# eezkni/UEGAN

Measured on AMD Instinct MI355X. Metric: train imgs/sec @512px bs=16 on 1/2/4/8 MI355X; infer ms/img, higher is better.
Workload: dtype bf16; 1 GPU; FiveK-shaped 512x512 batch=16/GPU, full G/D/VGG train step (trainer.py:77-119), conv_dim=32, seeded stand-in VGG19; global_batch=16, parallelism=dp1, pool_size=50, collective=none (1 rank), passes=batched (fused.py)

## Files before the change

uegan_amd/csrc/conv_core.h:

```cpp
#pragma once
#include "common.h"
#include "conv_internal.h"

#include <stdio.h>
#include <stdlib.h>
#include <utility>
#include <vector>

namespace uegan {

struct ProfRecord {
  hipEvent_t start, stop;
  int kernel_id;
  double flops, bytes;
};
extern bool g_prof_on;
extern std::vector<ProfRecord> g_prof_records;
extern std::vector<std::pair<hipEvent_t, hipEvent_t>> g_prof_pool;
extern size_t g_prof_used;

static inline int prof_key(int kind, bool bf16, int bn, int ks, int mode, int th, bool glds) {
  return (kind << 28) | ((bf16 ? 1 : 0) << 24) | (bn << 12) | (ks << 8) | (mode << 4) | ((th == 32 ? 2 : (th == 16 ? 1 : (th == 4 ? 3 : 0))) << 1) | (glds ? 1 : 0);
}
static void prof_kernel_name(int key, char* buf, size_t n) {
// ... 106 lines not shown
    if (o < out_n - 1 - g.pad || o > out_n - 2) return -1;
    pp = 2 * (out_n - 1) - o;
  }
  const int t2 = pp + g.pad - t;
  if (t2 < 0) return -1;
  int s = t2;
  if (g.stride == 2) {
    if (t2 & 1) return -1;
    s = t2 >> 1;
  }
  return s < in_n ? s : -1;
}

__device__ __forceinline__ bool has_image(const ConvGeom& g, int o, int img, int out_n) {
  if (img == 0) return true;
  if (g.mode == 0 || g.pad_mode != UEGAN_PAD_REFLECT) return false;
  if (img == 1) return o >= 1 && o <= g.pad;
  return o >= out_n - 1 - g.pad && o <= out_n - 2;
}

__device__ __forceinline__ int swz128(int r) { return ((r >> 1) & 3) << 1; }
__device__ __forceinline__ int swz64(int r) { return ((r >> 2) & 1) << 1; }

static __device__ __attribute__((aligned(16))) const unsigned int g_zero16[4] = {0u, 0u, 0u, 0u};

__device__ __forceinline__ void glds16(const void* gsrc, void* lds_wave_base) {
  __builtin_amdgcn_global_load_lds((const __attribute__((address_space(1))) void*)gsrc,
                                   (__attribute__((address_space(3))) void*)lds_wave_base, 16, 0, 0);
}

__device__ __forceinline__ void wgtr_glds16(const unsigned char* base, uint32_t off, unsigned char* lds_wave_base) {
#ifdef UEGAN_EMU
  glds16(base + off, lds_wave_base);
#else
  const uint32_t dst = (uint32_t)(uintptr_t)(__attribute__((address_space(3))) unsigned char*)lds_wave_base;
  uint32_t keep;
  asm volatile("s_mov_b32 %0, m0\n\ts_mov_b32 m0, %3\n\ts_nop 0\n\tglobal_load_lds_dwordx4 %1, %2\n\ts_mov_b32 m0, %0"
               : "=&s"(keep) : "v"(off), "s"(base), "s"(dst) : "memory");
#endif
}
__device__ __forceinline__ void wgtr_glds16(const void* src, unsigned char* lds_wave_base) {
#ifdef UEGAN_EMU
  glds16(src, lds_wave_base);
#else
  const uint32_t dst = (uint32_t)(uintptr_t)(__attribute__((address_space(3))) unsigned char*)lds_wave_base;
  uint32_t keep;
  asm volatile("s_mov_b32 %0, m0\n\ts_mov_b32 m0, %2\n\ts_nop 0\n\tglobal_load_lds_dwordx4 %1, off\n\ts_mov_b32 m0, %0"
               : "=&s"(keep) : "v"(src), "s"(dst) : "memory");
#endif
}
__device__ __forceinline__ void wgtr_wait_loads() {
#ifndef UEGAN_EMU
  asm volatile("s_waitcnt vmcnt(0)" ::: "memory");
#endif
}

struct ConvArgs {
  ConvGeom g;
  const void* in1;
  const void* in2;
  const void* w;
  const float* bias;
  const float* scale;
  int scale_group;
  void* out;
  void* out2;
  int n_out1;
  int N, Kp, act, nbias;
  int nty, ntx;
  int frame;
  int fy0, fy1, fx0, fx1;
  const void* mask;
  int mask_act;
  void* pool_out = nullptr;
  int pool_done = 0;
  void* pool_idx = nullptr;
  int n_idx = 0;
  int n_full = 1 << 30;
  int xcd_map = 0;
  int rect_y0 = 0, rect_y1 = 0, rect_x0 = 0, rect_x1 = 0;
  int border_only = 0;
  float* stats_part = nullptr;
  int stats_tpi = 0;
  const void* in1_lo = nullptr;
  const void* in2_lo = nullptr;
  const void* w_lo = nullptr;
  void* out_lo = nullptr;
  const void* mul = nullptr;
  const void* mul_lo = nullptr;
  void* out_mul = nullptr;
  void* out_mul_lo = nullptr;
  int src_wrap = 0;
  const float* res_x = nullptr;
  const float* res_x2 = nullptr;
  float* res_out = nullptr;
  float* res_out2 = nullptr;
  int res_split = 1 << 30;
  float* kws = nullptr;
  size_t kws_bytes = 0;
  int kparts = 0, kchunks = 0;
};

static inline int splitk_parts(const ConvArgs& a, int blocks, int nchunk, int* kchunks) {
  *kchunks = nchunk;
  if (!a.kws || a.g.mode != 0 || a.frame || a.out2 || a.mask || a.pool_out || a.stats_part || a.out_lo || a.mul || a.res_out || blocks <= 0) return 1;
  int parts = 1;
// ... 16 lines not shown
```

uegan_amd/csrc/conv_stream.h:

```cpp
#pragma once

struct ConvStreamArgs {
  ConvArgs c;
  int flip;
  int org;
  int zero_fill;
  int cls;
  int kstart[5];
  int ymin;
  int sx;
  int TH, PW, PH, PWmagic, KWmagic;
  int rb, rblog, Clog;
  int ksteps, taps;
  int wrow, wrows;
  int wbytes, tbytes, xbytes;
  int mtab_off;
  int xmir;
  int ty0, ty1, tx0, tx1;
  int tiles_total, tiles_per_block;
  int abl;
  int lo_xoff, c_lo, rb_lo, rblog_lo, wlo_off, tlo_off;
};

__device__ __forceinline__ int cs_swz(int rb, int pcol) {
  return rb == 128 ? swz128(pcol) : (rb == 64 ? swz64(pcol) : 0);
}

constexpr int CS_LDS_KB[4] = {53, 80, 152, 160};

template <int TN, int PF, int LC, bool CLS, bool XMIR = false, int NW = 4, bool STATS = false, int PR = 0, int EPX = 0>
__global__ void __launch_bounds__(64 * NW, (LC >= 2 ? 1 : (LC == 1 ? 2 : 3)) * NW / 4) conv_stream_kernel(ConvStreamArgs a) {
  constexpr int NT = 64 * NW;
  constexpr int MAXIX = (LC >= 2 ? 16 : 10) * 4 / NW;
  constexpr bool WLO = PR >= 1;
  static_assert(PR == 0 || (!CLS && !XMIR), "hi + lo pairs: plain forward only");
  __shared__ __attribute__((aligned(16))) unsigned char lds[CS_LDS_KB[LC] * 1024];
  const ConvArgs& ca = a.c;
  const ConvGeom& g = ca.g;
  const unsigned char* in1 = static_cast<const unsigned char*>(ca.in1);
  const unsigned char* in2 = static_cast<const unsigned char*>(ca.in2);
  const int tid = threadIdx.x, lane = tid & 63;
  const int wave = __builtin_amdgcn_readfirstlane(tid >> 6);
  const int fj = lane & 15, fg = lane >> 4;
  unsigned char* wl = lds;
  unsigned char* tab = lds + a.wbytes;
  unsigned char* xb0 = tab + a.tbytes;

  if (XMIR) {
    int* mflag = reinterpret_cast<int*>(tab + a.mtab_off) + 2 * a.ksteps * 64;
    for (int i = tid; i < 2 * a.ksteps; i += NT) mflag[i] = 0;
    __syncthreads();
  }
  {
    const int cpr = a.ksteps * 4;
    const int total = a.wrows * cpr;
    const bf16_t* w = static_cast<const bf16_t*>(ca.w);
    for (int idx = tid; idx < total; idx += NT) {
      const int n = idx / cpr, q = idx - n * cpr;
      u32x4 v = u32x4{0u, 0u, 0u, 0u};
      if (n < ca.N && q * 8 < ca.Kp) v = *reinterpret_cast<const u32x4*>(w + (size_t)n * ca.Kp + q * 8);
      *reinterpret_cast<u32x4*>(wl + n * a.wrow + (q >> 2) * 64 + (((q & 3) ^ swz64(n)) << 4)) = v;
      if constexpr (WLO) {
        u32x4 vl = u32x4{0u, 0u, 0u, 0u};
        if (n < ca.N && q * 8 < ca.Kp) vl = *reinterpret_cast<const u32x4*>(static_cast<const bf16_t*>(ca.w_lo) + (size_t)n * ca.Kp + q * 8);
        *reinterpret_cast<u32x4*>(wl + a.wlo_off + n * a.wrow + (q >> 2) * 64 + (((q & 3) ^ swz64(n)) << 4)) = vl;
      }
    }
    int* tab2 = reinterpret_cast<int*>(tab + a.ksteps * 256);
    if (!CLS) {
      for (int idx = tid; idx < a.ksteps * 64; idx += NT) {
        const int s = idx >> 6, l = idx & 63;
        const int k = 32 * s + 8 * (l >> 4);
        int tap = k >> a.Clog;
        const int chunk = (k & ((1 << a.Clog) - 1)) >> 3;
        if (tap >= a.taps) tap = 0;
        int ty = (tap * a.KWmagic) >> 16, tx = tap - ty * g.KW;
        if (a.flip) { ty = g.KH - 1 - ty; tx = g.KW - 1 - tx; }
        const int pcol = a.sx * (l & 15) + tx;
        *reinterpret_cast<int*>(tab + idx * 4) = (ty * a.PW + pcol) * a.rb + ((chunk ^ cs_swz(a.rb, pcol)) << 4);
        if (l == 0) tab2[s] = s * 64;
        if (XMIR) {
// ... 50 lines not shown
  const int nxc = (a.PH * a.PW) << cprlog;
  const int cprlog_lo = PR >= 2 ? a.rblog_lo - 4 : 0;
  const int nlo0 = PR >= 2 ? a.lo_xoff >> 4 : 0, nxcl = PR >= 2 ? (a.PH * a.PW) << cprlog_lo : 0;
  const int nix = PR >= 2 ? (nlo0 + nxcl + NT - 1) / NT : (nxc + NT - 1) / NT;
  const unsigned char* in_lo = PR == 2 ? static_cast<const unsigned char*>(ca.in1_lo) : (PR == 3 ? static_cast<const unsigned char*>(ca.in2_lo) : nullptr);
  const bool two_src = g.C2 != 0;
  auto decode = [&](int L, int& prow, int& pcol, int& c, int& sel) -> bool {
    if (PR >= 2 && L >= nlo0) {
      const int L2 = L - nlo0;
      if (L2 >= nxcl) return false;
      const int r = L2 >> cprlog_lo, pos = L2 & ((1 << cprlog_lo) - 1);
      prow = (r * a.PWmagic) >> 16; pcol = r - prow * a.PW;
      c = (pos ^ cs_swz(a.rb_lo, pcol)) << 3;
      sel = 2;
      return true;
    }
    if (PR >= 2 && L >= nxc) return false;
    const int r = L >> cprlog, pos = L & ((1 << cprlog) - 1);
    prow = (r * a.PWmagic) >> 16; pcol = r - prow * a.PW;
    c = (pos ^ cs_swz(a.rb, pcol)) << 3;
    sel = c < g.C1 ? 0 : 1;
    if (sel) c -= g.C1;
    return true;
  };
  uint32_t xoff[MAXIX];
#pragma unroll
  for (int it = 0; it < MAXIX; ++it) {
    const int L = it * NT + tid;
    xoff[it] = PR >= 2 ? 0xffffffffu : 0u;
    int prow, pcol, c, sel;
    if (L < (PR >= 2 ? nlo0 + nxcl : nxc) && decode(L, prow, pcol, c, sel)) {
      if (sel == 0) xoff[it] = (uint32_t)(((prow * g.IW + pcol) * g.C1 + c) * 2);
      else if (sel == 1) xoff[it] = (uint32_t)(((prow * g.IW + pcol) * g.C2 + c) * 2) | 0x80000000u;
      else xoff[it] = (uint32_t)(((prow * g.IW + pcol) * a.c_lo + c) * 2) | 0x40000000u;
    }
  }
  int abase[TN];
#pragma unroll
  for (int nf = 0; nf < TN; ++nf) {
    int n = nf * 16 + fj;
    if (n >= a.wrows) n -= a.wrows;
    abase[nf] = n * a.wrow + ((fg ^ swz64(n)) << 4);
  }
  float bv[TN][4];
#pragma unroll
  for (int nf = 0; nf < TN; ++nf)
#pragma unroll
    for (int r = 0; r < 4; ++r) {
      const int n = nf * 16 + fg * 4 + r;
      bv[nf][r] = (ca.bias && n < ca.nbias) ? ca.bias[n] : 0.f;
    }
  __syncthreads();

  const int nrx = a.tx1 - a.tx0, nry = a.ty1 - a.ty0;
  int t_begin = blockIdx.x * a.tiles_per_block, t_end = t_begin + a.tiles_per_block;
  if (t_end > a.tiles_total) t_end = a.tiles_total;

  auto tile_origin = [&](int t, int& b, int& oy0, int& ox0) {
    const int txi = t % nrx;
    const int tq = t / nrx;
    const int tyi = tq % nry;
    b = tq / nry;
    oy0 = (a.ty0 + tyi) * a.TH;
    ox0 = (a.tx0 + txi) * 16;
  };

  auto stage = [&](int t, int bufi) {
    unsigned char* xb = xb0 + bufi * a.xbytes;
    int b, oy0, ox0;
    tile_origin(t, b, oy0, ox0);
    const int iy0 = CLS ? oy0 + a.ymin : a.sx * oy0 + a.org, ix0 = CLS ? ox0 + a.ymin : a.sx * ox0 + a.org;
    const bool inside = iy0 >= 0 && iy0 + a.PH <= g.IH && ix0 >= 0 && ix0 + a.PW <= g.IW;
    if (inside) {
      const long long pix0 = ((long long)b * g.IH + iy0) * g.IW + ix0;
      const unsigned char* o1 = in1 + pix0 * g.C1 * 2;
      const unsigned char* o2 = in2 + pix0 * g.C2 * 2;
      const unsigned char* o3 = PR >= 2 ? in_lo + pix0 * a.c_lo * 2 : nullptr;
#pragma unroll
      for (int it = 0; it < MAXIX; ++it)
        if (it < nix) {
          const uint32_t o = xoff[it];
          unsigned char* dst = xb + (it * NT + wave * 64) * 16;
          if (PR >= 2 && o == 0xffffffffu) continue;
          if (PR >= 2 && (o & 0x40000000u)) wgtr_glds16(o3, o & 0x3fffffffu, dst);
          else if (two_src && (o >> 31)) wgtr_glds16(o2, o & 0x7fffffffu, dst);
          else wgtr_glds16(o1, o, dst);
        }
    } else if (!a.zero_fill) {
      const long long img = (long long)b * g.IH * g.IW;
      const unsigned char* o1 = in1 + img * g.C1 * 2;
      const unsigned char* o2 = in2 + img * g.C2 * 2;
      const unsigned char* o3 = PR >= 2 ? in_lo + img * a.c_lo * 2 : nullptr;
#pragma unroll 1
      for (int it = 0; it < nix; ++it) {
        const int L = it * NT + tid;
        int prow, pcol, c, sel;
        unsigned char* dst = xb + (it * NT + wave * 64) * 16;
        if (!decode(L, prow, pcol, c, sel)) continue;
        int iy = iy0 + prow, ix = ix0 + pcol;
        iy = iy < 0 ? -iy : iy;
        iy = iy >= g.IH ? 2 * (g.IH - 1) - iy : iy;
        iy = iy < 0 ? 0 : (iy >= g.IH ? g.IH - 1 : iy);
        ix = ix < 0 ? -ix : ix;
        ix = ix >= g.IW ? 2 * (g.IW - 1) - ix : ix;
        ix = ix < 0 ? 0 : (ix >= g.IW ? g.IW - 1 : ix);
        const uint32_t pix = (uint32_t)(iy * g.IW + ix);
        if (sel == 0) wgtr_glds16(o1, (pix * (uint32_t)g.C1 + (uint32_t)c) * 2u, dst);
        else if (sel == 1) wgtr_glds16(o2, (pix * (uint32_t)g.C2 + (uint32_t)c) * 2u, dst);
        else wgtr_glds16(o3, (pix * (uint32_t)a.c_lo + (uint32_t)c) * 2u, dst);
      }
    } else {
#pragma unroll 1
      for (int it = 0; it < nix; ++it) {
        const int L = it * NT + tid;
        const void* src = g_zero16;
        if (L < nxc) {
          const int r = L >> cprlog, pos = L & ((1 << cprlog) - 1);
          const int prow = (r * a.PWmagic) >> 16, pcol = r - prow * a.PW;
          const int c = (pos ^ cs_swz(a.rb, pcol)) << 3;
          const int iy = iy0 + prow, ix = ix0 + pcol;
          if (iy >= 0 && iy < g.IH && ix >= 0 && ix < g.IW) {
            const long long pix = ((long long)b * g.IH + iy) * g.IW + ix;
            src = c < g.C1 ? in1 + (pix * g.C1 + c) * 2 : in2 + (pix * g.C2 + (c - g.C1)) * 2;
          }
        }
        wgtr_glds16(src, xb + (it * NT + wave * 64) * 16);
      }
    }
  };

  bf16_t* out = static_cast<bf16_t*>(ca.out);
  float st1[STATS ? TN : 1][4], st2[STATS ? TN : 1][4];
  int st_b = -1;
  const int st_b0 = STATS ? t_begin / (ca.stats_tpi > 0 ? ca.stats_tpi : 1) : 0;
  if (STATS) {
#pragma unroll
    for (int nf = 0; nf < TN; ++nf)
#pragma unroll
      for (int r = 0; r < 4; ++r) { st1[nf][r] = 0.f; st2[nf][r] = 0.f; }
  }
  auto stats_flush = [&](int bimg) {
    if constexpr (STATS) {
      float* dst = ca.stats_part + ((size_t)((blockIdx.x * 2 + (bimg - st_b0)) * NW + wave) * (TN * 16)) * 2;
#pragma unroll
      for (int nf = 0; nf < TN; ++nf)
#pragma unroll
        for (int r = 0; r < 4; ++r) {
          float a1 = st1[nf][r], a2 = st2[nf][r];
#pragma unroll
          for (int o = 1; o < 16; o <<= 1) { a1 += __shfl_xor(a1, o, 64); a2 += __shfl_xor(a2, o, 64); }
          if (fj == 0) { dst[(nf * 16 + fg * 4 + r) * 2] = a1; dst[(nf * 16 + fg * 4 + r) * 2 + 1] = a2; }
          st1[nf][r] = 0.f; st2[nf][r] = 0.f;
        }
    }
  };
  const int row0 = wave * PF;
  int sc_grp = -1;
  float scale = 1.f;
  const int rowpitch = a.sx * a.PW * a.rb;
  for (int t = t_begin - 1; t < t_end; ++t) {
    const bool have = t >= t_begin;
    const int bufi = (t - t_begin) & 1;
    if (have) {
      wgtr_wait_loads();
      raw_barrier();
    }
    if (t + 1 < t_end && !((UEGAN_ABL_BITS(a.abl) & 1) && have)) stage(t + 1, bufi ^ 1);
    if (!have) continue;
    const unsigned char* xw = xb0 + bufi * a.xbytes + row0 * rowpitch;
    const int* tab2 = reinterpret_cast<const int*>(tab + a.ksteps * 256);
    constexpr int ncls = CLS ? 4 : 1;
   for (int cl = 0; cl < ncls; ++cl) {
    const int ks0 = CLS ? a.kstart[cl] : 0, ks1 = CLS ? a.kstart[cl + 1] : a.ksteps;
    f32x4 acc[TN][PF];
#pragma unroll
    for (int nf = 0; nf < TN; ++nf)
#pragma unroll
      for (int i = 0; i < PF; ++i) acc[nf][i] = f32x4{0.f, 0.f, 0.f, 0.f};
    u32x2 mulh[EPX == 2 ? TN : 1][EPX == 2 ? PF : 1], mull[EPX == 2 ? TN : 1][EPX == 2 ? PF : 1];
    if constexpr (EPX == 2) {
      int bq, oyq, oxq;
      tile_origin(t, bq, oyq, oxq);
#pragma unroll
      for (int i = 0; i < PF; ++i) {
        const int oy = oyq + row0 + i, oxp = oxq + fj;
        const bool pvq = oy < g.OH && oxp < g.OW;
        const size_t pq = ((size_t)bq * g.OH + oy) * g.OW + oxp;
#pragma unroll
        for (int nf = 0; nf < TN; ++nf) {
          mulh[nf][i] = u32x2{0u, 0u}; mull[nf][i] = u32x2{0u, 0u};
          if (pvq && nf * 16 + fg * 4 < ca.N) {
            const size_t eo = pq * ca.N + nf * 16 + fg * 4;
            mulh[nf][i] = *reinterpret_cast<const u32x2*>(static_cast<const bf16_t*>(ca.mul) + eo);
            if (ca.mul_lo) mull[nf][i] = *reinterpret_cast<const u32x2*>(static_cast<const bf16_t*>(ca.mul_lo) + eo);
          }
        }
      }
    }
    u32x4 a0[TN], b0[PF], a1[TN], b1[PF];
   if constexpr (PR != 0) {
    const int rowpitch_lo = a.sx * a.PW * a.rb_lo;
    const unsigned char* xwl = xb0 + bufi * a.xbytes + a.lo_xoff + row0 * rowpitch_lo;
    u32x4 al0[TN], al1[TN], bl0[PF], bl1[PF];
    auto load_p = [&](int s, auto odd_c, u32x4 (&af)[TN], u32x4 (&afl)[TN], u32x4 (&bf)[PF], u32x4 (&bfl)[PF]) {
      constexpr bool ODD = decltype(odd_c)::value;
      const int boff = *reinterpret_cast<const int*>(tab + (s * 64 + lane) * 4);
#pragma unroll
      for (int nf = 0; nf < TN; ++nf) {
        af[nf] = *reinterpret_cast<const u32x4*>(wl + abase[nf] + s * 64);
        afl[nf] = *reinterpret_cast<const u32x4*>(wl + a.wlo_off + abase[nf] + s * 64);
      }
#pragma unroll
      for (int i = 0; i < PF; ++i) bf[i] = *reinterpret_cast<const u32x4*>(xw + boff + i * rowpitch);
      if constexpr (PR == 2) {
#pragma unroll
        for (int i = 0; i < PF; ++i) bfl[i] = *reinterpret_cast<const u32x4*>(xwl + boff + i * rowpitch_lo);
      }
      if constexpr (PR == 3 && ODD) {
        const int bl = *reinterpret_cast<const int*>(tab + a.tlo_off + ((s >> 1) * 64 + lane) * 4);
#pragma unroll
        for (int i = 0; i < PF; ++i) bfl[i] = *reinterpret_cast<const u32x4*>(xwl + bl + i * rowpitch_lo);
      }
    };
    auto mma_p = [&](auto odd_c, const u32x4 (&af)[TN], const u32x4 (&afl)[TN], const u32x4 (&bf)[PF], const u32x4 (&bfl)[PF]) {
      constexpr bool ODD = decltype(odd_c)::value;
#pragma unroll
      for (int nf = 0; nf < TN; ++nf)
#pragma unroll
        for (int i = 0; i < PF; ++i) {
          if constexpr (PR == 2 || (PR == 3 && ODD)) acc[nf][i] = mfma_bf16(af[nf], bfl[i], acc[nf][i]);
          acc[nf][i] = mfma_bf16(afl[nf], bf[i], acc[nf][i]);
          acc[nf][i] = mfma_bf16(af[nf], bf[i], acc[nf][i]);
        }
    };
    const std::false_type even_c{};
    const std::true_type odd_c{};
    load_p(0, even_c, a0, al0, b0, bl0);
    for (int s = 0; s < ks1; s += 2) {
      if (s + 1 < ks1) load_p(s + 1, odd_c, a1, al1, b1, bl1);
      mma_p(even_c, a0, al0, b0, bl0);
      if (s + 1 >= ks1) break;
      if (s + 2 < ks1) load_p(s + 2, even_c, a0, al0, b0, bl0);
      mma_p(odd_c, a1, al1, b1, bl1);
    }
   } else {
    int boff_nx = *reinterpret_cast<const int*>(tab + (ks0 * 64 + lane) * 4);
    auto load_frags = [&](int s, u32x4 (&af)[TN], u32x4 (&bf)[PF]) {
      const int boff = boff_nx;
      if (s + 1 < ks1) boff_nx = *reinterpret_cast<const int*>(tab + ((s + 1) * 64 + lane) * 4);
      const int aoff = CLS ? tab2[s] : s * 64;
#pragma unroll
      for (int nf = 0; nf < TN; ++nf) af[nf] = *reinterpret_cast<const u32x4*>(wl + abase[nf] + aoff);
#pragma unroll
      for (int i = 0; i < PF; ++i) bf[i] = *reinterpret_cast<const u32x4*>(xw + boff + i * rowpitch);
    };
// ... 232 lines not shown
  int cspan = 0;
  for (int c = 0; c < 5; ++c) a.kstart[c] = 0;
  if (cls) {
    const int ymin = (g.pad & 1) ? (1 - g.pad) / 2 : -(g.pad / 2);
    int ymax = 0;
    for (int py = 0; py < 2; ++py) {
      const int t0 = (py + g.pad) & 1, v = (py + g.pad - t0) / 2;
      if (v > ymax) ymax = v;
    }
    a.ymin = ymin;
    cspan = ymax - ymin;
    a.PW = 16 + cspan;
    const int spt = g.C / 32;
    for (int c = 0; c < 4; ++c) {
      const int py = c >> 1, px = c & 1;
      const int nty = (g.KH - ((py + g.pad) & 1) + 1) / 2, ntx = (g.KW - ((px + g.pad) & 1) + 1) / 2;
      a.kstart[c + 1] = a.kstart[c] + nty * ntx * spt;
    }
    if (a.kstart[4] != a.ksteps) return false;
  }
  a.PWmagic = 65536 / a.PW + 1;
  p.pf = 0;
  p.lc = 1;
  for (int pass = 1; pass < (pr == 3 ? 4 : 3) && !p.pf; ++pass) {
    const int kb = CS_LDS_KB[pass], maxix = pass >= 2 ? 16 : 10;
    for (int pf : {4, 2}) {
      if (pf > max_pf) continue;
      const int th = 4 * pf, ph = cls ? th + cspan : sx * (th - 1) + g.KH;
      const int xbh = pr >= 2 ? ph * a.PW * a.rb : (ph * a.PW * a.rb + 4095) / 4096 * 4096;
      const int xb = xbh + (pr >= 2 ? ph * a.PW * a.rb_lo : 0);
      if (a.wbytes + a.tbytes + 2 * xb > kb * 1024 || (xb + 4095) / 4096 > maxix) continue;
      bool ok = true;
      for (int r = 0; r < ph * a.PW && ok; ++r) ok = ((r * a.PWmagic) >> 16) == r / a.PW;
      if (!ok) continue;
      p.pf = pf; a.TH = th; a.PH = ph; a.xbytes = xb; p.lc = pass;
      if (pr >= 2) a.lo_xoff = xbh;
      break;
    }
  }
  if (!p.pf) return false;
  p.nw = 4;
  if (p.pf == 4 && (!cls || p.lc == 2) && p.lc == 2 && p.tn <= 2 && !a.xmir && !pr) {
    const int xb8 = (a.PH * a.PW * a.rb + 8191) / 8192 * 8192;
    if (a.wbytes + a.tbytes + 2 * xb8 <= CS_LDS_KB[p.lc] * 1024 && xb8 / 8192 <= (p.lc == 2 ? 8 : 5)) { p.nw = 8; p.pf = 2; a.xbytes = xb8; }
  }
  if (pr >= 2 && p.lc >= 2 && p.tn <= 2 && (a.xbytes + 8191) / 8192 <= 8) { p.nw = 8; p.pf /= 2; }
  if (p.lc == 2 && ((p.tn == 4 && sx == 1) || (cls && p.nw != 8))) return false;
  p.fixup = g.mode == 1 && g.pad_mode == UEGAN_PAD_REFLECT && g.pad > 0;
  if (p.fixup && (g.OH <= 2 * g.pad + 2 || g.OW <= 2 * g.pad + 2)) return false;
  a.ty0 = 0; a.tx0 = 0;
  a.ty1 = ((cls ? g.IH : g.OH) + a.TH - 1) / a.TH;
  a.tx1 = ((cls ? g.IW : g.OW) + 15) / 16;
  a.tiles_total = g.B * (a.ty1 - a.ty0) * (a.tx1 - a.tx0);
  const int maxb = p.lc == 2 ? 256 : 512;
  int blocks = a.tiles_total < maxb ? a.tiles_total : maxb;
  a.tiles_per_block = (a.tiles_total + blocks - 1) / blocks;
  p.blocks = (a.tiles_total + a.tiles_per_block - 1) / a.tiles_per_block;
  if ((pr || epx) && !conv_stream_ex_available(p)) return false;
  return true;
}

template <int TN, int PF>
static void conv_stream_launch2(const ConvStreamPlan& p, hipStream_t s) {
  const int blocks = p.blocks;
  if (p.a.cls) {
    if constexpr (PF == 2 && TN <= 2) {
      if (p.nw == 8) {
        hipLaunchKernelGGL((conv_stream_kernel<TN, PF, 2, true, false, 8>), dim3(blocks), dim3(512), 0, s, p.a);
        return;
      }
    }
    if (p.lc == 2) hipLaunchKernelGGL((conv_stream_kernel<TN, PF, 2, true>), dim3(blocks), dim3(256), 0, s, p.a);
    else hipLaunchKernelGGL((conv_stream_kernel<TN, PF, 1, true>), dim3(blocks), dim3(256), 0, s, p.a);
    return;
  }
  if constexpr (PF == 2 && TN <= 2) {
    if (p.nw == 8) {
      if (p.a.xmir) hipLaunchKernelGGL((conv_stream_kernel<TN, PF, 1, false, true, 8>), dim3(blocks), dim3(512), 0, s, p.a);
      else if (p.lc == 2) hipLaunchKernelGGL((conv_stream_kernel<TN, PF, 2, false, false, 8>), dim3(blocks), dim3(512), 0, s, p.a);
      else hipLaunchKernelGGL((conv_stream_kernel<TN, PF, 1, false, false, 8>), dim3(blocks), dim3(512), 0, s, p.a);
      return;
    }
  }
  if (p.stats) {
    if constexpr (TN >= 2) {
      hipLaunchKernelGGL((conv_stream_kernel<TN, PF, 1, false, false, 4, true>), dim3(blocks), dim3(256), 0, s, p.a);
      return;
    }
  }
  if (p.a.xmir) {
    if (p.lc == 2) hipLaunchKernelGGL((conv_stream_kernel<TN, PF, 2, false, true>), dim3(blocks), dim3(256), 0, s, p.a);
    else hipLaunchKernelGGL((conv_stream_kernel<TN, PF, 1, false, true>), dim3(blocks), dim3(256), 0, s, p.a);
    return;
  }
  if (p.lc == 2) hipLaunchKernelGGL((conv_stream_kernel<TN, PF, 2, false>), dim3(blocks), dim3(256), 0, s, p.a);
  else hipLaunchKernelGGL((conv_stream_kernel<TN, PF, 1, false>), dim3(blocks), dim3(256), 0, s, p.a);
}
static bool conv_stream_stats_ok(const ConvStreamPlan& p) {
  const ConvGeom& g = p.a.c.g;
  const int tpi = (p.a.ty1 - p.a.ty0) * (p.a.tx1 - p.a.tx0);
  return g.mode == 0 && !p.a.cls && !p.a.xmir && p.nw == 4 && p.lc == 1 && !p.a.c.out2 && !p.a.c.mask && p.a.tiles_per_block <= tpi && p.tn >= 2;
}
static void conv_stream_launch(const ConvStreamPlan& p, hipStream_t s) {
  if (p.pr || p.epx) {
    (void)conv_stream_launch_ex(p, s);
    return;
// ... 10 lines not shown
```

uegan_amd/csrc/wgrad_tr.h:

```cpp
#pragma once

struct WgradTrArgs {
  ConvGeom g;
  const void* in1;
  const void* in2;
  const void* dz;
  float* ws;
  int N, zC, ktot, pstride, want_bias;
  int TW, TWlog, TH, PW, PWmagic, PWused, nks, dyk;
  int xrb, xrblog, zrb, zrblog;
  int xcb;
  int cfpc, fslots, fpb, nfr;
  int WK, WS;
  int tiles_x, tiles_y, tiles_total, tiles_per_split;
  int xbytes, zbytes;
  int rs;
  int nbuf;
  int xcd_map;
  int abl;
  int head, hE, hEB, hEBlog;
};

__device__ __forceinline__ int wgtr_swz(int rb, int r) {
  return rb == 128 ? (r & 6) : (rb == 64 ? ((r >> 1) & 2) : 0);
}

template <int KB>
__device__ __forceinline__ unsigned char* wgtr_lds() {
  __shared__ __attribute__((aligned(16))) unsigned char buf[KB * 1024];
  return buf;
}

__device__ __forceinline__ u32x2 lds_read_tr16(const unsigned char* p) {
  typedef short v4s_t __attribute__((ext_vector_type(4)));
  const v4s_t r = __builtin_amdgcn_ds_read_tr16_b64_v4i16((__attribute__((address_space(3))) v4s_t*)p);
  return __builtin_bit_cast(u32x2, r);
}

constexpr int WGTR_SMALL_KB = 80, WGTR_BIG_KB = 152;


template <int TN, int TM, bool BIG, bool HEAD>
__global__ void __launch_bounds__(256, BIG ? 1 : 2) wgrad_tr_kernel(WgradTrArgs a) {
  constexpr int MAXIX = BIG ? 19 : 10, MAXIZ = 8;
  unsigned char* lds = wgtr_lds<BIG ? WGTR_BIG_KB : WGTR_SMALL_KB>();
  const ConvGeom& g = a.g;
  const unsigned char* in1 = static_cast<const unsigned char*>(a.in1);
  const unsigned char* in2 = static_cast<const unsigned char*>(a.in2);
  const unsigned char* dz = static_cast<const unsigned char*>(a.dz);
  const int tid = threadIdx.x, lane = tid & 63;
  const int wave = __builtin_amdgcn_readfirstlane(tid >> 6);
  const int wk = wave % a.WK, wsid = wave / a.WK;
  int bx = blockIdx.x, by = blockIdx.y, bz = blockIdx.z;
  if (a.xcd_map) {
    const int P = gridDim.x * gridDim.y, G = a.xcd_map, m = 8 / G;
    const int L = blockIdx.x + gridDim.x * (blockIdx.y + gridDim.y * blockIdx.z);
    const int run = L / (G * P), r = L - run * G * P;
    const int xcd = r & 7, k = r >> 3;
    bz = run * G + xcd % G;
    const int q = k * m + xcd / G;
    by = q / gridDim.x;
    bx = q - by * gridDim.x;
  }
  const int cc = bx / a.nfr, fr = bx - cc * a.nfr;
  const int nb = by, split = bz;
  const int taps = g.KH * g.KW;
  const int f0 = fr * a.fpb;
  int tapA, tapB;
  if (a.cfpc) { tapA = f0 / a.cfpc; tapB = (f0 + a.fpb - 1) / a.cfpc; }
  else { tapA = 2 * f0; tapB = 2 * (f0 + a.fpb) - 1; }
  if (HEAD) { tapA *= g.KW; tapB = tapB * g.KW + g.KW - 1; }
  if (tapB > taps - 1) tapB = taps - 1;
  if (tapA > taps - 1) tapA = taps - 1;
  const int ty_lo = tapA / g.KW, ty_hi = tapB / g.KW;
  const int rstep = g.stride / a.rs;
  const int PH = (a.TH - 1) * rstep + (ty_hi - ty_lo) + 1;
  const int xcpr_log = a.xrblog - 4, zcpr_log = a.zrblog - 4;
  const int nxc = (PH * a.PW) << xcpr_log, nzc = (a.TH * a.TW) << zcpr_log;
  const int c_chunk0 = cc * 64, n_chunk0 = nb * 64;
  const int nix = (nxc + 255) >> 8, niz = (nzc + 255) >> 8;

  uint32_t xoff[MAXIX];
  const bool two_src = g.C2 != 0 && c_chunk0 < g.C1 && c_chunk0 + a.xcb > g.C1;
  const bool chunk_in2 = g.C2 != 0 && c_chunk0 >= g.C1;
#pragma unroll
  for (int it = 0; it < MAXIX; ++it) {
    const int L = it * 256 + tid;
    xoff[it] = 0;
    if (L < nxc) {
      const int r = L >> xcpr_log, pos = L & ((1 << xcpr_log) - 1);
      const int prow = (r * a.PWmagic) >> 16, pcol = r - prow * a.PW;
      const int c = c_chunk0 + ((pos ^ wgtr_swz(a.xrb, pcol)) << 3);
      if (pcol < a.PWused && c < g.C) {
        if (c < g.C1) xoff[it] = (uint32_t)(((prow * a.rs * g.IW + pcol) * g.C1 + c) * 2);
        else xoff[it] = (uint32_t)(((prow * a.rs * g.IW + pcol) * g.C2 + (c - g.C1)) * 2) | (two_src ? 0x80000000u : 0u);
      }
    }
  }
  uint32_t zoff[MAXIZ];
#pragma unroll
  for (int it = 0; it < MAXIZ; ++it) {
    const int L = it * 256 + tid;
    zoff[it] = 0;
    if (L < nzc) {
      const int r = L >> zcpr_log, pos = L & ((1 << zcpr_log) - 1);
      const int oy = r >> a.TWlog, ox = r & (a.TW - 1);
      const int c = n_chunk0 + ((pos ^ wgtr_swz(a.zrb, r)) << 3);
      if (c < a.zC) zoff[it] = (uint32_t)(((oy * g.OW + ox) * a.zC + c) * 2);
    }
  }

  const int g4 = lane >> 4, sj = (lane & 15) >> 2, seg = lane & 3;
  const int dx = sj + 4 * (g4 & 1) + (a.TW == 32 ? 16 * (g4 >> 1) : 0);
  const int dy = a.TW == 32 ? 0 : (g4 >> 1);
  int zaddr[TN], xaddr[TM], xaddr1[TM];
  if (HEAD) {
    const int zch = a.hEB >> 1;
#pragma unroll
    for (int nf = 0; nf < TN; ++nf) {
      int ch = nf * 16 + 4 * seg;
      if (ch >= zch) ch = 4 * (seg & 1);
      zaddr[nf] = dx * a.hEB + ((((ch >> 3) ^ wgtr_swz(a.hEB, dx))) << 4) + ((ch >> 2) & 1) * 8;
    }
#pragma unroll
    for (int m = 0; m < TM; ++m) {
      const int f = f0 + wk * TM + m;
      int ty = f / a.cfpc;
      const int ch = (f - ty * a.cfpc) * 16 + 4 * seg;
      if (ty > ty_hi) ty = ty_lo;
      const int q1 = dx + 32 < a.PWused ? dx + 32 : a.PWused - 1;
      xaddr[m] = ((ty - ty_lo) * a.PW + dx) * a.xrb + ((((ch >> 3) ^ wgtr_swz(a.xrb, dx))) << 4) + ((ch >> 2) & 1) * 8;
      xaddr1[m] = ((ty - ty_lo) * a.PW + q1) * a.xrb + ((((ch >> 3) ^ wgtr_swz(a.xrb, q1))) << 4) + ((ch >> 2) & 1) * 8;
    }
  } else {
#pragma unroll
    for (int m = 0; m < TM; ++m) xaddr1[m] = 0;
    const int rz = dy * a.TW + dx;
    const int zcb = a.zC - n_chunk0 < 64 ? a.zC - n_chunk0 : 64;
#pragma unroll
    for (int nf = 0; nf < TN; ++nf) {
      int ch = nf * 16 + 4 * seg;
      if (ch >= zcb) ch = 4 * (seg & 1);
      zaddr[nf] = rz * a.zrb + ((((ch >> 3) ^ wgtr_swz(a.zrb, rz))) << 4) + ((ch >> 2) & 1) * 8;
    }
#pragma unroll
    for (int m = 0; m < TM; ++m) {
      const int f = f0 + wk * TM + m;
      int tap, ch;
      if (a.cfpc) { tap = f / a.cfpc; ch = (f - tap * a.cfpc) * 16 + 4 * seg; }
      else { tap = 2 * f + (seg >> 1); ch = 4 * (seg & 1); }
      if (tap > tapB) tap = tapA;
      const int ty = tap / g.KW, tx = tap - ty * g.KW;
      const int pcx = dx * g.stride + tx;
      const int rx = (dy * rstep + ty - ty_lo) * a.PW + pcx;
      xaddr[m] = rx * a.xrb + ((((ch >> 3) ^ wgtr_swz(a.xrb, pcx))) << 4) + ((ch >> 2) & 1) * 8;
    }
  }
  const int z_ks = HEAD ? 32 * a.hEB : a.dyk * a.TW * a.zrb, z_h = 8 * (HEAD ? a.hEB : a.zrb);
  const int x_ks = a.dyk * rstep * a.PW * a.xrb, x_h = 8 * g.stride * a.xrb;
  unsigned char* const dzx = lds + 2 * (a.xbytes + a.zbytes);

  f32x4 acc[TN][TM];
#pragma unroll
  for (int i = 0; i < TN; ++i)
#pragma unroll
    for (int m = 0; m < TM; ++m) acc[i][m] = f32x4{0.f, 0.f, 0.f, 0.f};

  f32x4 accb[TN];
#pragma unroll
  for (int i = 0; i < TN; ++i) accb[i] = f32x4{0.f, 0.f, 0.f, 0.f};
  const bool do_bias = a.want_bias && bx == 0 && wk == 0;
  const uint32_t one2 = (uint32_t)f32_to_bf16(1.f) * 0x10001u;
  const u32x4 ones = u32x4{one2, one2, one2, one2};

  int t_begin = split * a.tiles_per_split, t_end = t_begin + a.tiles_per_split;
  if (t_end > a.tiles_total) t_end = a.tiles_total;

  auto stage = [&](int t, int bufi) {
    unsigned char* xb = lds + bufi * (a.xbytes + a.zbytes);
    unsigned char* zb = xb + a.xbytes;
    const int txi = t % a.tiles_x;
    const int tq = t / a.tiles_x;
    const int tyi = tq % a.tiles_y, b = tq / a.tiles_y;
    const int oy0 = tyi * a.TH, ox0 = txi * a.TW;
    const int iy0 = oy0 * g.stride + ty_lo - g.pad, ix0 = ox0 * g.stride - g.pad;
    const bool z_inside = oy0 + a.TH <= g.OH && ox0 + a.TW <= g.OW;
    const bool x_inside = iy0 >= 0 && iy0 + (PH - 1) * a.rs + 1 <= g.IH && ix0 >= 0 && ix0 + a.PWused <= g.IW;
    if (x_inside && z_inside) {
      const long long pix0 = ((long long)b * g.IH + iy0) * g.IW + ix0;
      const unsigned char* o2 = in2 + pix0 * g.C2 * 2;
      const unsigned char* o1 = chunk_in2 ? o2 : in1 + pix0 * g.C1 * 2;
#pragma unroll
      for (int it = 0; it < MAXIX; ++it)
        if (it < nix) {
          const uint32_t o = xoff[it];
          unsigned char* dst = xb + (it * 256 + wave * 64) * 16;
          if (two_src && (o >> 31)) wgtr_glds16(o2, o & 0x7fffffffu, dst);
          else wgtr_glds16(o1, o, dst);
        }
    } else if (g.pad_mode == UEGAN_PAD_REFLECT) {
      const long long img = (long long)b * g.IH * g.IW;
      const unsigned char* o2 = in2 + img * g.C2 * 2;
// ... 90 lines not shown
              hw[tx * NN + n] = (n & 1) ? (word >> 16) : (word & 0xffffu);
            }
          }
          unsigned char* dst = dzx + pq * a.hEB;
          const int sw = wgtr_swz(a.hEB, q);
#pragma unroll
          for (int c = 0; c < 4; ++c)
            if (c < cpp)
              *reinterpret_cast<u32x4*>(dst + ((c ^ sw) << 4)) = u32x4{hw[8 * c] | (hw[8 * c + 1] << 16), hw[8 * c + 2] | (hw[8 * c + 3] << 16),
                                                                        hw[8 * c + 4] | (hw[8 * c + 5] << 16), hw[8 * c + 6] | (hw[8 * c + 7] << 16)};
        }
      };
      if (!(UEGAN_ABL_BITS(a.abl) & 8))
      switch (a.N) {
        case 1: build(std::integral_constant<int, 1>{}); break;
        case 2: build(std::integral_constant<int, 2>{}); break;
        case 3: build(std::integral_constant<int, 3>{}); break;
        default: build(std::integral_constant<int, 4>{}); break;
      }
      __syncthreads();
    }
    for (int ks = wsid; ks < ((UEGAN_ABL_BITS(a.abl) & 2) ? 0 : a.nks); ks += a.WS) {
      const unsigned char* zk = HEAD ? dzx + ks * z_ks : zb + ks * z_ks;
      const unsigned char* xk = HEAD ? xb + (ks >> 1) * a.PW * a.xrb : xb + ks * x_ks;
      const bool half1 = HEAD && (ks & 1);
      constexpr int PD0 = TN >= 4 ? 2 : (TN == 2 ? 4 : 8), PD = PD0 < TM ? PD0 : TM;
      u32x4 af[TN], bf[PD];
      auto read_x = [&](int m) {
        const int xa = half1 ? xaddr1[m] : xaddr[m];
        const u32x2 lo = lds_read_tr16(xk + xa), hi = lds_read_tr16(xk + (half1 ? xa : xa + x_h));
        return u32x4{lo.x, lo.y, hi.x, hi.y};
      };
#pragma unroll
      for (int nf = 0; nf < TN; ++nf) {
        const u32x2 lo = lds_read_tr16(zk + zaddr[nf]), hi = lds_read_tr16(zk + zaddr[nf] + z_h);
        af[nf] = u32x4{lo.x, lo.y, hi.x, hi.y};
      }
#pragma unroll
      for (int m = 0; m < PD; ++m) bf[m] = read_x(m);
      if (do_bias) {
#pragma unroll
        for (int nf = 0; nf < TN; ++nf) accb[nf] = mfma_bf16(af[nf], ones, accb[nf]);
      }
#pragma unroll
      for (int m = 0; m < TM; ++m) {
        const u32x4 b = bf[m % PD];
        if (m + PD < TM) bf[m % PD] = read_x(m + PD);
#pragma unroll
        for (int nf = 0; nf < TN; ++nf) acc[nf][m] = mfma_bf16(af[nf], b, acc[nf][m]);
      }
    }
  }

  float* ws = a.ws + (size_t)(split * a.WS + wsid) * a.pstride;
  const int col = lane & 15;
  if (do_bias && col == 0) {
#pragma unroll
    for (int nf = 0; nf < TN; ++nf)
#pragma unroll
      for (int r = 0; r < 4; ++r) {
        const int n = n_chunk0 + nf * 16 + (lane >> 4) * 4 + r;
        if (n < a.N) ws[(size_t)a.N * a.ktot + n] = accb[nf][r];
      }
  }
  if (HEAD) {
#pragma unroll
    for (int m = 0; m < TM; ++m) {
      const int f = f0 + wk * TM + m;
      const int ty = f / a.cfpc;
      if (ty >= g.KH) continue;
      const int kc = c_chunk0 + (f - ty * a.cfpc) * 16 + col;
#pragma unroll
      for (int nf = 0; nf < TN; ++nf)
#pragma unroll
        for (int r = 0; r < 4; ++r) {
          const int i = nf * 16 + (lane >> 4) * 4 + r;
          if (i >= a.hE) continue;
          const int tx = i / a.N, n = i - tx * a.N;
          ws[(size_t)n * a.ktot + (ty * g.KW + tx) * g.C + kc] = acc[nf][m][r];
        }
    }
    return;
  }
#pragma unroll
  for (int m = 0; m < TM; ++m) {
    const int f = f0 + wk * TM + m;
    int tap, kk;
    if (a.cfpc) { tap = f / a.cfpc; kk = tap * g.C + c_chunk0 + (f - tap * a.cfpc) * 16 + col; }
    else { tap = 2 * f + (col >> 3); kk = tap * g.C + (col & 7); }
    if (tap >= taps) continue;
#pragma unroll
    for (int nf = 0; nf < TN; ++nf)
#pragma unroll
      for (int r = 0; r < 4; ++r) {
        const int n = n_chunk0 + nf * 16 + (lane >> 4) * 4 + r;
        if (n < a.N) ws[(size_t)n * a.ktot + kk] = acc[nf][m][r];
      }
  }
}

static bool g_use_wgtr = true;

struct WgradTrPlan {
  WgradTrArgs a;
  dim3 grid;
  int nsplit_eff;
  int tn, tm;
  bool big;
};

static bool wgtr_ch_ok(int c) { return c == 8 || c == 16 || c == 32 || (c >= 64 && c % 64 == 0); }

static bool wgtr_plan(const uegan_conv_desc* d, const ConvGeom& g, WgradTrPlan& p) {
  if (!g_use_wgtr || d->dtype != UEGAN_BF16) return false;
  const int C = d->C1 + d->C2, zC = d->Cout;
  if (!wgtr_ch_ok(C) || !wgtr_ch_ok(zC)) return false;
  if (C < 64 && d->C2 != 0) {  }
  WgradTrArgs& a = p.a;
  a.g = g;
  a.abl = UEGAN_ABL_BITS(g_abl_stream);
  a.N = d->Cout_w ? d->Cout_w : d->Cout;
  a.zC = zC;
  a.ktot = d->KH * d->KW * C;
  a.pstride = a.N * a.ktot + a.N;
  a.want_bias = 1;
  const int s = d->stride;
  a.head = 0; a.hE = 0; a.hEB = 16; a.hEBlog = 4;
  if (a.N <= 4 && zC == 8 && s == 1 && d->KW >= 3 && d->KW <= 7 && d->Wo >= 32 && C >= 16) {
    a.head = 1;
    a.hE = d->KW * a.N;
    a.hEB = a.hE <= 8 ? 16 : (a.hE <= 16 ? 32 : 64);
    a.hEBlog = a.hEB == 16 ? 4 : (a.hEB == 32 ? 5 : 6);
  }
  a.TW = (s == 1 && d->Wo >= 32 && (a.head || (d->KH == 1 && d->KW == 1))) ? 32 : 16;
  a.TWlog = a.TW == 32 ? 5 : 4;
  a.dyk = a.TW == 32 ? 1 : 2;
  a.PWused = (a.TW - 1) * s + d->KW;
  a.PW = a.PWused;
  a.PWmagic = 65536 / a.PW + 1;
  a.xcb = C < 64 ? C : 64;
  a.xrb = a.xcb * 2;
  const int zcb = zC < 64 ? zC : 64;
  a.zrb = zcb * 2;
  a.xrblog = a.xrb == 128 ? 7 : (a.xrb == 64 ? 6 : (a.xrb == 32 ? 5 : 4));
  a.zrblog = a.zrb == 128 ? 7 : (a.zrb == 64 ? 6 : (a.zrb == 32 ? 5 : 4));
  const int taps = d->KH * d->KW;
  a.cfpc = a.xcb >= 16 ? a.xcb / 16 : 0;
  a.fslots = a.head ? d->KH * a.cfpc : (a.cfpc ? taps * a.cfpc : (taps + 1) / 2);
  const int F = a.fslots;
  static const int tms[7] = {1, 2, 3, 4, 5, 7, 9};
  if (F >= 20) {
    a.WK = 4;
    int best = 0, best_slots = 1 << 30;
    for (int tm : {9, 7, 5}) {
      const int slots = (F + 4 * tm - 1) / (4 * tm) * 4 * tm;
      if (slots < best_slots) { best_slots = slots; best = tm; }
    }
    p.tm = best;
  } else {
    a.WK = F > 9 ? 2 : 1;
    const int need = (F + a.WK - 1) / a.WK;
    p.tm = 9;
    for (int tm : tms)
      if (tm >= need) { p.tm = tm; break; }
  }
  a.WS = 4 / a.WK;
  a.fpb = a.WK * p.tm;
  a.nfr = (F + a.fpb - 1) / a.fpb;
  int krows = d->KH;
  if (!a.head && a.cfpc) {
    krows = 1;
    for (int fr = 0; fr < a.nfr; ++fr) {
      const int tA = fr * a.fpb / a.cfpc;
      int tB = (fr * a.fpb + a.fpb - 1) / a.cfpc;
      if (tB > taps - 1) tB = taps - 1;
      const int span = tB / d->KW - tA / d->KW + 1;
      if (span > krows) krows = span;
    }
  }
  a.rs = (s == 2 && krows == 1) ? 2 : 1;
  const int rstep = s / a.rs;
  static const int th32[4] = {8, 4, 2, 1}, th16[4] = {16, 8, 4, 2};
  const int* ths = a.TW == 32 ? th32 : th16;
  int cap = ths[3];
  while (cap < d->Ho && cap < ths[0]) cap *= 2;
  auto dzx_bytes = [&](int th) { return a.head ? (th * 64 * a.hEB + 4095) / 4096 * 4096 : 0; };
  auto bytes = [&](int th, int& xb, int& zb) {
    xb = (((th - 1) * rstep + krows) * a.PW * a.xrb + 4095) / 4096 * 4096;
    zb = (th * a.TW * a.zrb + 4095) / 4096 * 4096;
    return 2 * (xb + zb);
  };
  auto fits = [&](int th, int kb) {
    int xb, zb;
    return th <= cap && bytes(th, xb, zb) + dzx_bytes(th) <= kb * 1024;
  };
  a.TH = 0;
  a.nbuf = 2;
  p.big = false;
  for (int i = 0; i < 4 && !a.TH; ++i)
    if (fits(ths[i], WGTR_SMALL_KB)) a.TH = ths[i];
  if (!a.TH) {
    p.big = true;
    for (int i = 0; i < 4 && !a.TH; ++i)
      if (fits(ths[i], WGTR_BIG_KB)) a.TH = ths[i];
  }
  if (!a.TH) return false;
  a.nks = a.head ? 2 * a.TH : a.TH / a.dyk;
  bytes(a.TH, a.xbytes, a.zbytes);
  {
    const int rows = ((a.TH - 1) * rstep + krows) * a.PW;
    for (int r = 0; r < rows; ++r)
      if (((r * a.PWmagic) >> 16) != r / a.PW) return false;
    const int nix = ((rows * a.xrb / 16) + 255) / 256, niz = ((a.TH * a.TW * a.zrb / 16) + 255) / 256;
    if (nix > (p.big ? 19 : 10) || niz > 8) return false;
  }
  p.tn = zcb >= 64 ? 4 : (zcb >= 32 ? 2 : 1);
  if (a.head) p.tn = a.hE <= 16 ? 1 : 2;
  const int cchunks = (C + 63) / 64, nblk = (zC + 63) / 64;
  a.tiles_x = (d->Wo + a.TW - 1) / a.TW;
  a.tiles_y = (d->Ho + a.TH - 1) / a.TH;
  a.tiles_total = d->B * a.tiles_x * a.tiles_y;
  const int per_split = cchunks * a.nfr * nblk;
  constexpr int target = 512;
  int want = (target + per_split - 1) / per_split;
  if (want < 1) want = 1;
  if (want > 8 && g_tuning[UEGAN_TUNE_WGRAD_XCD] != 0) want = (want + 7) / 8 * 8;
  if (want > a.tiles_total) want = a.tiles_total;
  a.tiles_per_split = (a.tiles_total + want - 1) / want;
  const int nsplit = (a.tiles_total + a.tiles_per_split - 1) / a.tiles_per_split;
  p.nsplit_eff = nsplit * a.WS;
  p.grid = dim3(cchunks * a.nfr, nblk, nsplit);
  a.xcd_map = 0;
  if (per_split > 1 && g_tuning[UEGAN_TUNE_WGRAD_XCD] != 0) {
    if (nsplit % 8 == 0) a.xcd_map = 8;
    else if ((nsplit == 1 || nsplit == 2 || nsplit == 4) && (nsplit * per_split) % 8 == 0 && per_split % (8 / nsplit) == 0) a.xcd_map = nsplit;
  }
  return true;
}

template <int TN, int TM>
static void wgtr_launch2(const WgradTrPlan& p, hipStream_t s) {
  if (p.a.head) {
    if constexpr (TN <= 2) {
      if (p.big) hipLaunchKernelGGL((wgrad_tr_kernel<TN, TM, true, true>), p.grid, dim3(256), 0, s, p.a);
      else hipLaunchKernelGGL((wgrad_tr_kernel<TN, TM, false, true>), p.grid, dim3(256), 0, s, p.a);
    }
    return;
  }
  if (p.big) hipLaunchKernelGGL((wgrad_tr_kernel<TN, TM, true, false>), p.grid, dim3(256), 0, s, p.a);
  else hipLaunchKernelGGL((wgrad_tr_kernel<TN, TM, false, false>), p.grid, dim3(256), 0, s, p.a);
}
template <int TN>
static void wgtr_launch1(const WgradTrPlan& p, hipStream_t s) {
  switch (p.tm) {
    case 1: wgtr_launch2<TN, 1>(p, s); break;
    case 2: wgtr_launch2<TN, 2>(p, s); break;
    case 3: wgtr_launch2<TN, 3>(p, s); break;
    case 4: wgtr_launch2<TN, 4>(p, s); break;
    case 5: wgtr_launch2<TN, 5>(p, s); break;
    case 7: wgtr_launch2<TN, 7>(p, s); break;
    default: wgtr_launch2<TN, 9>(p, s); break;
  }
}
static void wgtr_launch(const WgradTrPlan& p, hipStream_t s) {
  if (p.tn == 1) wgtr_launch1<1>(p, s);
  else if (p.tn == 2) wgtr_launch1<2>(p, s);
  else wgtr_launch1<4>(p, s);
}
```

Measured before the change: 501.8 imgs/sec.

## Deepen conv stream input staging to N-buffer ring with partial vmcnt waits

```diff
diff --git a/uegan_amd/csrc/conv_core.h b/uegan_amd/csrc/conv_core.h
--- a/uegan_amd/csrc/conv_core.h
+++ b/uegan_amd/csrc/conv_core.h
@@ -182,6 +182,23 @@
 __device__ __forceinline__ void wgtr_wait_loads() {
 #ifndef UEGAN_EMU
   asm volatile("s_waitcnt vmcnt(0)" ::: "memory");
+#endif
+}
+template <int LO, int HI>
+__device__ __forceinline__ void wgtr_wait_loads_le_r(int n) {
+  if constexpr (LO == HI) {
+    asm volatile("s_waitcnt vmcnt(%0)" ::"n"(LO) : "memory");
+  } else {
+    constexpr int M = (LO + HI + 1) / 2;
+    if (n >= M) wgtr_wait_loads_le_r<M, HI>(n);
+    else wgtr_wait_loads_le_r<LO, M - 1>(n);
+  }
+}
+__device__ __forceinline__ void wgtr_wait_loads_le(int n) {
+#ifndef UEGAN_EMU
+  wgtr_wait_loads_le_r<0, 63>(__builtin_amdgcn_readfirstlane(n));
+#else
+  (void)n;
 #endif
 }
 
diff --git a/uegan_amd/csrc/conv_stream.h b/uegan_amd/csrc/conv_stream.h
--- a/uegan_amd/csrc/conv_stream.h
+++ b/uegan_amd/csrc/conv_stream.h
@@ -18,6 +18,7 @@
   int xmir;
   int ty0, ty1, tx0, tx1;
   int tiles_total, tiles_per_block;
+  int nbuf;
   int abl;
   int lo_xoff, c_lo, rb_lo, rblog_lo, wlo_off, tlo_off;
 };
@@ -27,6 +28,7 @@
 }
 
 constexpr int CS_LDS_KB[4] = {53, 80, 152, 160};
+constexpr int CS_MAX_NBUF = 4;
 
 template <int TN, int PF, int LC, bool CLS, bool XMIR = false, int NW = 4, bool STATS = false, int PR = 0, int EPX = 0>
 __global__ void __launch_bounds__(64 * NW, (LC >= 2 ? 1 : (LC == 1 ? 2 : 3)) * NW / 4) conv_stream_kernel(ConvStreamArgs a) {
@@ -183,6 +185,15 @@
     }
   __syncthreads();
 
+  int nld = nix;
+  if constexpr (PR >= 2) {
+    nld = 0;
+    for (int it = 0; it < nix; ++it) {
+      const int L0 = it * NT + wave * 64;
+      if (L0 < nxc || (L0 + 64 > nlo0 && L0 < nlo0 + nxcl)) ++nld;
+    }
+  }
+
   const int nrx = a.tx1 - a.tx0, nry = a.ty1 - a.ty0;
   int t_begin = blockIdx.x * a.tiles_per_block, t_end = t_begin + a.tiles_per_block;
   if (t_end > a.tiles_total) t_end = a.tiles_total;
@@ -289,16 +300,21 @@
   int sc_grp = -1;
   float scale = 1.f;
   const int rowpitch = a.sx * a.PW * a.rb;
-  for (int t = t_begin - 1; t < t_end; ++t) {
+  const int nb1 = a.nbuf - 1;
+  int bufi = 0, sbuf = 0;
+  for (int t = t_begin - nb1; t < t_end; ++t) {
     const bool have = t >= t_begin;
-    const int bufi = (t - t_begin) & 1;
     if (have) {
-      wgtr_wait_loads();
+      const int younger = t_end - 1 - t < nb1 - 1 ? t_end - 1 - t : nb1 - 1;
+      wgtr_wait_loads_le(younger * nld);
       raw_barrier();
     }
-    if (t + 1 < t_end && !((UEGAN_ABL_BITS(a.abl) & 1) && have)) stage(t + 1, bufi ^ 1);
+    if (t + nb1 < t_end && !((UEGAN_ABL_BITS(a.abl) & 1) && have)) stage(t + nb1, sbuf);
+    if (++sbuf == a.nbuf) sbuf = 0;
     if (!have) continue;
-    const unsigned char* xw = xb0 + bufi * a.xbytes + row0 * rowpitch;
+    const int bufc = bufi;
+    if (++bufi == a.nbuf) bufi = 0;
+    const unsigned char* xw = xb0 + bufc * a.xbytes + row0 * rowpitch;
     const int* tab2 = reinterpret_cast<const int*>(tab + a.ksteps * 256);
     constexpr int ncls = CLS ? 4 : 1;
    for (int cl = 0; cl < ncls; ++cl) {
@@ -331,7 +347,7 @@
     u32x4 a0[TN], b0[PF], a1[TN], b1[PF];
    if constexpr (PR != 0) {
     const int rowpitch_lo = a.sx * a.PW * a.rb_lo;
-    const unsigned char* xwl = xb0 + bufi * a.xbytes + a.lo_xoff + row0 * rowpitch_lo;
+    const unsigned char* xwl = xb0 + bufc * a.xbytes + a.lo_xoff + row0 * rowpitch_lo;
     u32x4 al0[TN], al1[TN], bl0[PF], bl1[PF];
     auto load_p = [&](int s, auto odd_c, u32x4 (&af)[TN], u32x4 (&afl)[TN], u32x4 (&bf)[PF], u32x4 (&bfl)[PF]) {
       constexpr bool ODD = decltype(odd_c)::value;
@@ -670,6 +686,9 @@
   a.ty1 = ((cls ? g.IH : g.OH) + a.TH - 1) / a.TH;
   a.tx1 = ((cls ? g.IW : g.OW) + 15) / 16;
   a.tiles_total = g.B * (a.ty1 - a.ty0) * (a.tx1 - a.tx0);
+  a.nbuf = (CS_LDS_KB[p.lc] * 1024 - a.wbytes - a.tbytes) / a.xbytes;
+  if (a.nbuf > CS_MAX_NBUF) a.nbuf = CS_MAX_NBUF;
+  if (a.nbuf < 2) return false;
   const int maxb = p.lc == 2 ? 256 : 512;
   int blocks = a.tiles_total < maxb ? a.tiles_total : maxb;
   a.tiles_per_block = (a.tiles_total + blocks - 1) / blocks;
```

Result: no change. 497.8 imgs/sec, median of 2 (-0.8%).

## Reduce intra-block wave splits in LDS and pack four taps per slot for tiny-C wgrad

Applied to the files above, without the earlier changes.

```diff
diff --git a/uegan_amd/csrc/wgrad_tr.h b/uegan_amd/csrc/wgrad_tr.h
--- a/uegan_amd/csrc/wgrad_tr.h
+++ b/uegan_amd/csrc/wgrad_tr.h
@@ -11,6 +11,7 @@
   int xrb, xrblog, zrb, zrblog;
   int xcb;
   int cfpc, fslots, fpb, nfr;
+  int dense4;
   int WK, WS;
   int tiles_x, tiles_y, tiles_total, tiles_per_split;
   int xbytes, zbytes;
@@ -68,6 +69,7 @@
   const int f0 = fr * a.fpb;
   int tapA, tapB;
   if (a.cfpc) { tapA = f0 / a.cfpc; tapB = (f0 + a.fpb - 1) / a.cfpc; }
+  else if (a.dense4) { tapA = 4 * f0; tapB = 4 * (f0 + a.fpb) - 1; }
   else { tapA = 2 * f0; tapB = 2 * (f0 + a.fpb) - 1; }
   if (HEAD) { tapA *= g.KW; tapB = tapB * g.KW + g.KW - 1; }
   if (tapB > taps - 1) tapB = taps - 1;
@@ -148,6 +150,7 @@
       const int f = f0 + wk * TM + m;
       int tap, ch;
       if (a.cfpc) { tap = f / a.cfpc; ch = (f - tap * a.cfpc) * 16 + 4 * seg; }
+      else if (a.dense4) { tap = 4 * f + seg; ch = 0; }
       else { tap = 2 * f + (seg >> 1); ch = 4 * (seg & 1); }
       if (tap > tapB) tap = tapA;
       const int ty = tap / g.KW, tx = tap - ty * g.KW;
@@ -344,7 +347,43 @@
     }
   }
 
-  float* ws = a.ws + (size_t)(split * a.WS + wsid) * a.pstride;
+  if (a.WS > 1) {
+    float* red = reinterpret_cast<float*>(lds) + wk * (TN * TM + TN) * 256 + lane;
+    __syncthreads();
+    for (int w = 0; w < wsid; ++w) __syncthreads();
+    if (wsid > 0) {
+#pragma unroll
+      for (int nf = 0; nf < TN; ++nf)
+#pragma unroll
+        for (int m = 0; m < TM; ++m)
+#pragma unroll
+          for (int r = 0; r < 4; ++r) acc[nf][m][r] = red[((nf * TM + m) * 4 + r) * 64] + acc[nf][m][r];
+      if (do_bias) {
+#pragma unroll
+        for (int nf = 0; nf < TN; ++nf)
+#pragma unroll
+          for (int r = 0; r < 4; ++r) accb[nf][r] = red[((TN * TM + nf) * 4 + r) * 64] + accb[nf][r];
+      }
+    }
+    if (wsid < a.WS - 1) {
+#pragma unroll
+      for (int nf = 0; nf < TN; ++nf)
+#pragma unroll
+        for (int m = 0; m < TM; ++m)
+#pragma unroll
+          for (int r = 0; r < 4; ++r) red[((nf * TM + m) * 4 + r) * 64] = acc[nf][m][r];
+      if (do_bias) {
+#pragma unroll
+        for (int nf = 0; nf < TN; ++nf)
+#pragma unroll
+          for (int r = 0; r < 4; ++r) red[((TN * TM + nf) * 4 + r) * 64] = accb[nf][r];
+      }
+    }
+    for (int w = wsid; w < a.WS - 1; ++w) __syncthreads();
+    if (wsid != a.WS - 1) return;
+  }
+
+  float* ws = a.ws + (size_t)split * a.pstride;
   const int col = lane & 15;
   if (do_bias && col == 0) {
 #pragma unroll
@@ -379,6 +418,7 @@
     const int f = f0 + wk * TM + m;
     int tap, kk;
     if (a.cfpc) { tap = f / a.cfpc; kk = tap * g.C + c_chunk0 + (f - tap * a.cfpc) * 16 + col; }
+    else if (a.dense4) { tap = 4 * f + (col >> 2); kk = tap * g.C + (col & 3); }
     else { tap = 2 * f + (col >> 3); kk = tap * g.C + (col & 7); }
     if (tap >= taps) continue;
 #pragma unroll
@@ -438,7 +478,8 @@
   a.zrblog = a.zrb == 128 ? 7 : (a.zrb == 64 ? 6 : (a.zrb == 32 ? 5 : 4));
   const int taps = d->KH * d->KW;
   a.cfpc = a.xcb >= 16 ? a.xcb / 16 : 0;
-  a.fslots = a.head ? d->KH * a.cfpc : (a.cfpc ? taps * a.cfpc : (taps + 1) / 2);
+  a.dense4 = (a.cfpc == 0 && !a.head && d->C2 == 0 && (d->Cin_w ? d->Cin_w : C) <= 4) ? 1 : 0;
+  a.fslots = a.head ? d->KH * a.cfpc : (a.cfpc ? taps * a.cfpc : (a.dense4 ? (taps + 3) / 4 : (taps + 1) / 2));
   const int F = a.fslots;
   static const int tms[7] = {1, 2, 3, 4, 5, 7, 9};
   if (F >= 20) {
@@ -508,6 +549,7 @@
   }
   p.tn = zcb >= 64 ? 4 : (zcb >= 32 ? 2 : 1);
   if (a.head) p.tn = a.hE <= 16 ? 1 : 2;
+  if (a.WS > 1 && a.WK * (p.tn * p.tm + p.tn) * 1024 > (p.big ? WGTR_BIG_KB : WGTR_SMALL_KB) * 1024) return false;
   const int cchunks = (C + 63) / 64, nblk = (zC + 63) / 64;
   a.tiles_x = (d->Wo + a.TW - 1) / a.TW;
   a.tiles_y = (d->Ho + a.TH - 1) / a.TH;
@@ -520,7 +562,7 @@
   if (want > a.tiles_total) want = a.tiles_total;
   a.tiles_per_split = (a.tiles_total + want - 1) / want;
   const int nsplit = (a.tiles_total + a.tiles_per_split - 1) / a.tiles_per_split;
-  p.nsplit_eff = nsplit * a.WS;
+  p.nsplit_eff = nsplit;
   p.grid = dim3(cchunks * a.nfr, nblk, nsplit);
   a.xcd_map = 0;
   if (per_split > 1 && g_tuning[UEGAN_TUNE_WGRAD_XCD] != 0) {
```

Result: no change. 495.6 imgs/sec before, 494.7 imgs/sec after, median of 2 (-0.2%).
